# fdb/frequensea

Measured on AMD Instinct MI355X. Metric: fft_frames_per_sec_n8192, higher is better.
Workload: dtype f32

## Files before the change

### frequensea_amd/csrc/fsea_configs.h

```cpp
#pragma once

#include "fsea_opt.h"

#define FSEA_CFG_32 32, 4, 64, 2, 2, 8, 4, 1, 1, true, true, 0, fo::STREAMING_PIXELS | fo::WIN_DC_REGS
#define FSEA_CFG_64 64, 4, 64, 2, 2, 16, 4, 1, 1, true, true, 0, fo::STREAMING_PIXELS | fo::WIN_DC_REGS
#define FSEA_CFG_128 128, 4, 64, 2, 2, 16, 8, 1, 1, true, true, 0, fo::STREAMING_PIXELS | fo::WIN_DC_REGS
#define FSEA_CFG_256 256, 8, 32, 2, 2, 16, 16, 1, 1, true, true, 0, fo::STREAMING_PIXELS | fo::WIN_DC_REGS
#define FSEA_CFG_512 512, 16, 16, 2, 2, 32, 16, 1, 1, true, true, 0, fo::STREAMING_PIXELS | fo::WIN_DC_REGS
#define FSEA_CFG_1024 1024, 32, 8, 2, 3, 8, 16, 8, 1, true, true, 0, fo::STREAMING_PIXELS | fo::BALANCE_MAG | fo::WIN_DC_REGS_MAG | fo::LD_NT | fo::DEFER | fo::LANE_ROT | fo::TW_FUSE | fo::TW_HOIST | fo::BATCH_READS
#define FSEA_CFG_2048 2048, 64, 4, 2, 3, 16, 16, 8, 1, true, true, 0, fo::STREAMING_PIXELS | fo::BALANCE_MAG | fo::WIN_DC_REGS_MAG | fo::LD_NT | fo::LANE_ROT | fo::TW_FUSE | fo::TW_HOIST | fo::BATCH_READS
#define FSEA_CFG_4096 4096, 128, 2, 2, 3, 16, 16, 16, 1, true, true, 0, fo::STREAMING_PIXELS | fo::BALANCE_MAG | fo::LD_NT | fo::DEFER | fo::LANE_ROT_LAST | fo::LANE_ROT | fo::TW_FUSE | fo::TW_HOIST | fo::BATCH_READS
#define FSEA_CFG_8192 8192, 256, 1, 2, 3, 16, 16, 32, 1, true, true, 0, fo::STREAMING_PIXELS | fo::BALANCE_MAG | fo::WIN_DC_REGS | fo::LD_NT | fo::DEFER | fo::LANE_ROT | fo::TW_FUSE | fo::TW_HOIST | fo::BATCH_READS
#define FSEA_CFG_16384 16384, 512, 1, 2, 3, 16, 32, 32, 1, true, true, 0, fo::STREAMING_PIXELS | fo::WIN_DC_REGS_MAG | fo::LD_NT | fo::DEFER | fo::TW_FUSE

#define FSEA_CFG_256_ROWS 256, 8, 32, 2, 3, 4, 8, 8, 1, true, true, 0, fo::STREAMING_PIXELS | fo::WIN_DC_REGS | fo::LD_NT | fo::DEFER | fo::LANE_ROT | fo::TW_FUSE | fo::TW_HOIST | fo::BATCH_READS
#define FSEA_CFG_512_PX 512, 16, 16, 2, 2, 16, 32, 1, 1, true, true, 0, fo::STREAMING_PIXELS | fo::WIN_DC_REGS | fo::LD_NT | fo::TW_FUSE | fo::BATCH_READS
#define FSEA_CFG_1024_RT 1024, 32, 8, 2, 2, 32, 32, 1, 1, true, true, 0, fo::STREAMING_PIXELS | fo::WIN_DC_REGS | fo::TW_FUSE | fo::BATCH_READS

#define FSEA_WIN 2
```

### frequensea_amd/csrc/fsea_configs_tune.h

```cpp
#pragma once

#include "fsea_configs.h"

#define FSEA_CFG_8192_ND 8192, 256, 1, 2, 3, 16, 16, 32, 1, true, true, 0, fo::LANE_ROT | fo::TW_FUSE | fo::TW_HOIST | fo::BATCH_READS
#define FSEA_CFG_16384_ND 16384, 512, 1, 2, 3, 16, 32, 32, 1, true, true, 0, fo::TW_FUSE
#define FSEA_CFG_4096_DF 4096, 256, 1, 4, 3, 16, 16, 16, 1, true, true, 0, fo::DEFER | fo::TW_FUSE | fo::BATCH_READS
#define FSEA_CFG_2048_DF 2048, 64, 4, 2, 3, 16, 16, 8, 1, true, true, 0, fo::DEFER | fo::TW_FUSE | fo::TW_HOIST | fo::BATCH_READS
#define FSEA_CFG_8192_CP0 8192, 256, 1, 2, 3, 16, 16, 32, 1, true, true, 0, fo::DEFER | fo::LANE_ROT | fo::TW_FUSE | fo::TW_HOIST | fo::BATCH_READS
#define FSEA_CFG_8192_STNT 8192, 256, 1, 2, 3, 16, 16, 32, 1, true, true, 0, fo::ST_NT | fo::DEFER | fo::LANE_ROT | fo::TW_FUSE | fo::TW_HOIST | fo::BATCH_READS
#define FSEA_CFG_8192_LDNT 8192, 256, 1, 2, 3, 16, 16, 32, 1, true, true, 0, fo::LD_NT | fo::DEFER | fo::LANE_ROT | fo::TW_FUSE | fo::TW_HOIST | fo::BATCH_READS
#define FSEA_CFG_16384_CP0 16384, 512, 1, 2, 3, 16, 32, 32, 1, true, true, 0, fo::DEFER | fo::TW_FUSE
#define FSEA_CFG_16384_STNT 16384, 512, 1, 2, 3, 16, 32, 32, 1, true, true, 0, fo::ST_NT | fo::DEFER | fo::TW_FUSE
#define FSEA_CFG_4096_CP0 4096, 128, 2, 2, 3, 16, 16, 16, 1, true, true, 0, fo::DEFER | fo::LANE_ROT | fo::TW_FUSE | fo::TW_HOIST | fo::BATCH_READS
#define FSEA_CFG_4096_STNT 4096, 128, 2, 2, 3, 16, 16, 16, 1, true, true, 0, fo::ST_NT | fo::DEFER | fo::LANE_ROT | fo::TW_FUSE | fo::TW_HOIST | fo::BATCH_READS
#define FSEA_CFG_2048_CP0 2048, 64, 4, 2, 3, 16, 16, 8, 1, true, true, 0, fo::TW_FUSE | fo::TW_HOIST | fo::BATCH_READS
#define FSEA_CFG_2048_STNT 2048, 64, 4, 2, 3, 16, 16, 8, 1, true, true, 0, fo::ST_NT | fo::TW_FUSE | fo::TW_HOIST | fo::BATCH_READS
#define FSEA_CFG_1024_CP0 1024, 32, 8, 2, 2, 32, 32, 1, 1, true, true, 0, fo::TW_FUSE | fo::BATCH_READS
#define FSEA_CFG_1024_LDSTNT 1024, 32, 8, 2, 2, 32, 32, 1, 1, true, true, 0, fo::LD_NT | fo::ST_NT | fo::TW_FUSE | fo::BATCH_READS
#define FSEA_CFG_256_CP0 256, 8, 32, 2, 2, 16, 16, 1, 1, true, true, 0, 0
#define FSEA_CFG_256_LDSTNT 256, 8, 32, 2, 2, 16, 16, 1, 1, true, true, 0, fo::LD_NT | fo::ST_NT
#define FSEA_CFG_8192_V2 8192, 256, 1, 2, 3, 16, 16, 32, 1, true, true, 0, fo::V2 | fo::TW_FUSE | fo::BATCH_READS
#define FSEA_CFG_8192_V2S 8192, 256, 1, 2, 3, 16, 16, 32, 1, true, true, fsea::abl::V2_STATIC, fo::V2 | fo::TW_FUSE | fo::BATCH_READS
#define FSEA_CFG_8192_V2L 8192, 256, 1, 2, 3, 16, 16, 32, 1, true, true, fsea::abl::V2_V1_LOADS, fo::V2 | fo::TW_FUSE | fo::BATCH_READS
#define FSEA_CFG_8192_V2SL 8192, 256, 1, 2, 3, 16, 16, 32, 1, true, true, fsea::abl::V2_V1_LOADS | fsea::abl::V2_STATIC, fo::V2 | fo::TW_FUSE | fo::BATCH_READS
#define FSEA_CFG_8192_V2NA 8192, 256, 1, 2, 3, 16, 16, 32, 1, true, true, fsea::abl::V2_NO_EXCHANGE_A, fo::V2 | fo::TW_FUSE | fo::BATCH_READS
#define FSEA_CFG_8192_B2 8192, 256, 1, 2, 3, 16, 32, 16, 1, true, true, 0, fo::LD_NT | fo::ST_NT | fo::DEFER | fo::LANE_ROT | fo::TW_FUSE | fo::TW_HOIST | fo::BATCH_READS
#define FSEA_CFG_8192_D2 8192, 256, 1, 2, 3, 8, 32, 32, 1, true, true, 0, fo::LD_NT | fo::ST_NT | fo::DEFER | fo::LANE_ROT | fo::TW_FUSE | fo::TW_HOIST | fo::BATCH_READS
#define FSEA_CFG_8192_W 8192, 256, 1, 2, 3, 32, 32, 8, 1, true, true, 0, fo::LD_NT | fo::ST_NT | fo::DEFER | fo::LANE_ROT | fo::TW_FUSE | fo::TW_HOIST | fo::BATCH_READS
#define FSEA_CFG_8192_W2 8192, 256, 1, 2, 3, 32, 32, 8, 1, true, true, 0, fo::ST_NT | fo::DEFER | fo::LANE_ROT | fo::TW_FUSE | fo::TW_HOIST | fo::BATCH_READS
#define FSEA_CFG_8192_A 8192, 256, 1, 2, 3, 32, 16, 16, 1, true, true
#define FSEA_CFG_8192_B 8192, 256, 1, 2, 3, 16, 32, 16, 1, true, true
#define FSEA_CFG_8192_D 8192, 256, 1, 2, 3, 8, 32, 32, 1, true, true
#define FSEA_CFG_8192_NOTWL 8192, 256, 1, 2, 3, 16, 32, 16, 1, false, true
#define FSEA_CFG_8192_NOTWR 8192, 256, 1, 2, 3, 16, 32, 16, 1, true, false
#define FSEA_CFG_1024_B 1024, 64, 4, 4, 3, 16, 16, 4, 1, true, true
#define FSEA_CFG_1024_C 1024, 64, 4, 4, 3, 4, 16, 16, 1, true, true
#define FSEA_CFG_1024_D 1024, 32, 4, 2, 2, 32, 32, 1, 1, true, true
#define FSEA_CFG_4096_B 4096, 128, 2, 2, 3, 16, 16, 16, 1, true, true
#define FSEA_CFG_4096_C 4096, 128, 2, 2, 3, 16, 8, 32, 1, true, true
#define FSEA_CFG_4096_D 4096, 128, 2, 2, 3, 8, 16, 32, 1, true, true
#define FSEA_CFG_256_P16 256, 16, 16, 2, 2, 16, 16, 1, 1, true, true, 0, fo::ST_NT
#define FSEA_CFG_128_P16 128, 8, 32, 2, 2, 16, 8, 1, 1, true, true, 0, fo::ST_NT
#define FSEA_CFG_4096_T256 4096, 256, 1, 4, 3, 16, 16, 16, 1, true, true, 0, fo::LD_NT | fo::ST_NT | fo::TW_FUSE | fo::BATCH_READS
#define FSEA_CFG_4096_F1 4096, 128, 1, 2, 3, 16, 16, 16, 1, true, true, 0, fo::LD_NT | fo::ST_NT | fo::DEFER | fo::LANE_ROT | fo::TW_FUSE | fo::TW_HOIST | fo::BATCH_READS
#define FSEA_CFG_4096_B3 4096, 128, 2, 2, 3, 16, 16, 16, 1, true, true, 0, fo::LD_NT | fo::ST_NT | fo::LANE_ROT | fo::TW_FUSE | fo::TW_HOIST | fo::BATCH_READS
#define FSEA_CFG_4096_LR 4096, 128, 2, 2, 3, 16, 16, 16, 1, true, true, 0, fo::LD_NT | fo::ST_NT | fo::DEFER | fo::LANE_ROT | fo::TW_FUSE | fo::TW_HOIST | fo::BATCH_READS
#define FSEA_CFG_2048_LR 2048, 64, 4, 2, 3, 16, 16, 8, 1, true, true, 0, fo::LD_NT | fo::ST_NT | fo::TW_FUSE | fo::TW_HOIST | fo::BATCH_READS
#define FSEA_CFG_16384_B 16384, 512, 1, 2, 3, 32, 32, 16, 1, true, true
#define FSEA_CFG_2048_B 2048, 64, 4, 2, 3, 8, 8, 32, 1, true, true
#define FSEA_CFG_2048_C 2048, 64, 4, 2, 3, 4, 16, 32, 1, true, true
#define FSEA_CFG_8192_NOST 8192, 256, 1, 2, 3, 16, 16, 32, 1, true, true, fsea::abl::NO_STORES, fo::LANE_ROT | fo::TW_FUSE | fo::TW_HOIST | fo::BATCH_READS
#define FSEA_CFG_8192_NOLDS 8192, 256, 1, 2, 3, 16, 16, 32, 1, true, true, fsea::abl::NO_LDS, fo::LANE_ROT | fo::TW_FUSE | fo::TW_HOIST | fo::BATCH_READS
#define FSEA_CFG_8192_NOFLOP 8192, 256, 1, 2, 3, 16, 16, 32, 1, true, true, fsea::abl::NO_FLOPS, fo::LANE_ROT | fo::TW_FUSE | fo::TW_HOIST | fo::BATCH_READS
#define FSEA_CFG_8192_IO 8192, 256, 1, 2, 3, 16, 16, 32, 1, true, true, fsea::abl::NO_FLOPS | fsea::abl::NO_LDS, fo::LANE_ROT | fo::TW_FUSE | fo::TW_HOIST | fo::BATCH_READS
#define FSEA_CFG_8192_VALU 8192, 256, 1, 2, 3, 16, 16, 32, 1, true, true, fsea::abl::NO_LDS | fsea::abl::NO_STORES, fo::LANE_ROT | fo::TW_FUSE | fo::TW_HOIST | fo::BATCH_READS
#define FSEA_CFG_8192_IONT 8192, 256, 1, 2, 3, 16, 16, 32, 1, true, true, fsea::abl::NO_FLOPS | fsea::abl::NO_LDS, fo::LD_NT | fo::ST_NT | fo::LANE_ROT | fo::TW_FUSE | fo::TW_HOIST | fo::BATCH_READS
#define FSEA_CFG_8192_NOLDSNT 8192, 256, 1, 2, 3, 16, 16, 32, 1, true, true, fsea::abl::NO_LDS, fo::LD_NT | fo::ST_NT | fo::LANE_ROT | fo::TW_FUSE | fo::TW_HOIST | fo::BATCH_READS
#define FSEA_CFG_8192_NOFLOPNT 8192, 256, 1, 2, 3, 16, 16, 32, 1, true, true, fsea::abl::NO_FLOPS, fo::LD_NT | fo::ST_NT | fo::LANE_ROT | fo::TW_FUSE | fo::TW_HOIST | fo::BATCH_READS
#define FSEA_CFG_8192_NOLOAD 8192, 256, 1, 2, 3, 16, 16, 32, 1, true, true, fsea::abl::NO_LOADS, fo::LANE_ROT | fo::TW_FUSE | fo::TW_HOIST | fo::BATCH_READS
#define FSEA_CFG_128_ST0 128, 4, 64, 2, 2, 16, 8, 1, 1, true, true, 0, 0
#define FSEA_CFG_256_ST0 256, 8, 32, 2, 2, 16, 16, 1, 1, true, true, 0, 0
#define FSEA_CFG_512_ST0 512, 16, 16, 2, 2, 32, 16, 1, 1, true, true, 0, 0
#define FSEA_CFG_1024_ST0 1024, 32, 8, 2, 2, 32, 32, 1, 1, true, true, 0, fo::TW_FUSE | fo::BATCH_READS
#define FSEA_CFG_4096_PXNOLOG 4096, 128, 2, 2, 3, 16, 16, 16, 1, true, true, fsea::abl::NO_EPILOGUE_MATH, fo::LD_NT | fo::ST_NT | fo::DEFER | fo::LANE_ROT | fo::TW_FUSE | fo::TW_HOIST | fo::BATCH_READS
#define FSEA_CFG_4096_PXNOST 4096, 128, 2, 2, 3, 16, 16, 16, 1, true, true, fsea::abl::NO_STORES, fo::LD_NT | fo::ST_NT | fo::DEFER | fo::LANE_ROT | fo::TW_FUSE | fo::TW_HOIST | fo::BATCH_READS
#define FSEA_CFG_4096_PXIO 4096, 128, 2, 2, 3, 16, 16, 16, 1, true, true, fsea::abl::NO_FLOPS | fsea::abl::NO_LDS, fo::LD_NT | fo::ST_NT | fo::LANE_ROT | fo::TW_FUSE | fo::TW_HOIST | fo::BATCH_READS
#define FSEA_CFG_8192_PXNOLOG 8192, 256, 1, 2, 3, 16, 16, 32, 1, true, true, fsea::abl::NO_EPILOGUE_MATH, fo::LD_NT | fo::ST_NT | fo::DEFER | fo::LANE_ROT | fo::TW_FUSE | fo::TW_HOIST | fo::BATCH_READS
#define FSEA_CFG_8192_NOMAG 8192, 256, 1, 2, 3, 16, 16, 32, 1, true, true, fsea::abl::NO_EPILOGUE_MATH, fo::LANE_ROT | fo::TW_FUSE | fo::TW_HOIST | fo::BATCH_READS
#define FSEA_CFG_8192_X0 8192, 256, 1, 2, 3, 16, 16, 32, 1, true, true, 0, 0
#define FSEA_CFG_4096_X0 4096, 128, 2, 2, 3, 16, 16, 16, 1, true, true, 0, 0
#define FSEA_CFG_2048_X0 2048, 64, 4, 2, 3, 16, 16, 8, 1, true, true, 0, 0
#define FSEA_CFG_1024_X0 1024, 32, 8, 2, 2, 32, 32, 1, 1, true, true, 0, 0
#define FSEA_CFG_4096_W64 4096, 64, 1, 1, 2, 64, 64, 1, 1, false, false, 0, fo::W64 | fo::LD_NT | fo::ST_NT | fo::BATCH_READS
#define FSEA_CFG_4096_S2 4096, 64, 1, 1, 3, 16, 16, 16, 1, true, true, 0, fo::LD_NT | fo::ST_NT | fo::DEFER | fo::LANE_ROT | fo::TW_FUSE | fo::TW_HOIST | fo::BATCH_READS
#define FSEA_CFG_4096_W64B 4096, 64, 1, 1, 2, 64, 64, 1, 1, false, false, 0, fo::PX_BIAS | fo::W64 | fo::LD_NT | fo::ST_NT | fo::BATCH_READS
#define FSEA_CFG_4096_PK 4096, 128, 2, 2, 3, 16, 16, 16, 1, true, true, 0, fo::PX_PACK | fo::LD_NT | fo::ST_NT | fo::DEFER | fo::LANE_ROT_LAST | fo::LANE_ROT | fo::TW_FUSE | fo::TW_HOIST | fo::BATCH_READS
#define FSEA_CFG_4096_PX0 4096, 128, 2, 2, 3, 16, 16, 16, 1, true, true, 0, fo::LD_NT | fo::ST_NT | fo::DEFER | fo::LANE_ROT_LAST | fo::LANE_ROT | fo::TW_FUSE | fo::TW_HOIST | fo::BATCH_READS
#define FSEA_CFG_8192_PK 8192, 256, 1, 2, 3, 16, 16, 32, 1, true, true, 0, fo::PX_PACK | fo::LD_NT | fo::ST_NT | fo::DEFER | fo::LANE_ROT | fo::TW_FUSE | fo::TW_HOIST | fo::BATCH_READS
#define FSEA_CFG_8192_PX0 8192, 256, 1, 2, 3, 16, 16, 32, 1, true, true, 0, fo::LD_NT | fo::ST_NT | fo::DEFER | fo::LANE_ROT | fo::TW_FUSE | fo::TW_HOIST | fo::BATCH_READS
#define FSEA_CFG_256_PK 256, 8, 32, 2, 2, 16, 16, 1, 1, true, true, 0, fo::PX_PACK | fo::ST_NT
#define FSEA_CFG_256_PX0 256, 8, 32, 2, 2, 16, 16, 1, 1, true, true, 0, fo::ST_NT
#define FSEA_CFG_1024_PX0 1024, 32, 8, 2, 2, 32, 32, 1, 1, true, true, 0, fo::ST_NT | fo::TW_FUSE | fo::BATCH_READS
#define FSEA_CFG_1024_R2 FSEA_CFG_1024_RT
#define FSEA_CFG_256_P64 256, 4, 16, 1, 2, 16, 16, 1, 1, true, true, 0, fo::ST_NT
#define FSEA_CFG_4096_T256PX 4096, 256, 1, 4, 3, 16, 16, 16, 1, true, true, 0, fo::STREAMING_PIXELS | fo::LD_NT | fo::TW_FUSE | fo::BATCH_READS
#define FSEA_CFG_4096_F1PX 4096, 128, 1, 2, 3, 16, 16, 16, 1, true, true, 0, fo::STREAMING_PIXELS | fo::LD_NT | fo::DEFER | fo::LANE_ROT | fo::TW_FUSE | fo::TW_HOIST | fo::BATCH_READS
#define FSEA_CFG_32_C2 32, 4, 64, 2, 2, 4, 8, 1, 1, true, true, 0, fo::STREAMING_PIXELS
#define FSEA_CFG_64_C2 64, 4, 64, 2, 2, 8, 8, 1, 1, true, true, 0, fo::STREAMING_PIXELS
#define FSEA_CFG_64_T2 64, 2, 128, 2, 2, 8, 8, 1, 1, true, true, 0, fo::STREAMING_PIXELS
#define FSEA_CFG_1024_E 1024, 32, 8, 2, 3, 16, 8, 8, 1, true, true, 0, fo::STREAMING_PIXELS | fo::LD_NT | fo::LANE_ROT | fo::TW_FUSE | fo::TW_HOIST | fo::BATCH_READS
#define FSEA_CFG_1024_F 1024, 32, 8, 2, 3, 8, 16, 8, 1, true, true, 0, fo::STREAMING_PIXELS | fo::LD_NT | fo::LANE_ROT | fo::TW_FUSE | fo::TW_HOIST | fo::BATCH_READS
#define FSEA_CFG_1024_G 1024, 32, 8, 2, 3, 16, 16, 4, 1, true, true, 0, fo::STREAMING_PIXELS | fo::LD_NT | fo::LANE_ROT | fo::TW_FUSE | fo::TW_HOIST | fo::BATCH_READS
#define FSEA_CFG_1024_H 1024, 32, 8, 2, 3, 8, 8, 16, 1, true, true, 0, fo::STREAMING_PIXELS | fo::LD_NT | fo::LANE_ROT | fo::TW_FUSE | fo::TW_HOIST | fo::BATCH_READS
#define FSEA_CFG_1024_FD 1024, 32, 8, 2, 3, 8, 16, 8, 1, true, true, 0, fo::STREAMING_PIXELS | fo::LD_NT | fo::DEFER | fo::LANE_ROT | fo::TW_FUSE | fo::TW_HOIST | fo::BATCH_READS
#define FSEA_CFG_1024_F0 1024, 32, 8, 2, 3, 8, 16, 8, 1, true, true, 0, fo::STREAMING_PIXELS | fo::LD_NT | fo::TW_FUSE | fo::TW_HOIST | fo::BATCH_READS
#define FSEA_CFG_1024_FL 1024, 32, 8, 2, 3, 8, 16, 8, 1, true, true, 0, fo::STREAMING_PIXELS | fo::LANE_ROT | fo::TW_FUSE | fo::TW_HOIST | fo::BATCH_READS
#define FSEA_CFG_512_888 512, 16, 16, 2, 3, 8, 8, 8, 1, true, true, 0, fo::STREAMING_PIXELS | fo::LD_NT | fo::DEFER | fo::LANE_ROT | fo::TW_FUSE | fo::TW_HOIST | fo::BATCH_READS
#define FSEA_CFG_512_1632 FSEA_CFG_512_PX
#define FSEA_CFG_256_488 FSEA_CFG_256_ROWS
#define FSEA_CFG_256_884 256, 8, 32, 2, 3, 8, 8, 4, 1, true, true, 0, fo::STREAMING_PIXELS | fo::LD_NT | fo::DEFER | fo::LANE_ROT | fo::TW_FUSE | fo::TW_HOIST | fo::BATCH_READS
#define FSEA_CFG_128_448 128, 4, 64, 2, 3, 4, 4, 8, 1, true, true, 0, fo::STREAMING_PIXELS | fo::LD_NT | fo::DEFER | fo::LANE_ROT | fo::TW_FUSE | fo::TW_HOIST | fo::BATCH_READS
#define FSEA_CFG_2048_81616 2048, 64, 4, 2, 3, 8, 16, 16, 1, true, true, 0, fo::STREAMING_PIXELS | fo::LD_NT | fo::DEFER | fo::LANE_ROT | fo::TW_FUSE | fo::TW_HOIST | fo::BATCH_READS
#define FSEA_CFG_4096_16328 4096, 128, 2, 2, 3, 16, 32, 8, 1, true, true, 0, fo::STREAMING_PIXELS | fo::LD_NT | fo::DEFER | fo::LANE_ROT_LAST | fo::LANE_ROT | fo::TW_FUSE | fo::TW_HOIST | fo::BATCH_READS
// ... 13 lines not shown
```

### frequensea_amd/csrc/fsea_fft_core.h

```cpp
#pragma once

#include <hip/hip_runtime.h>
#include <stddef.h>
#include <stdint.h>

#include <fsea_pk_asm.h>
#include "fsea_opt.h"
#ifdef FSEA_TUNE
#include <fsea_pk_asm_tune.h>
#endif

namespace fsea {

constexpr int ilog2c(int n) {
    int l = 0;
    while ((1 << l) < n) ++l;
    return l;
}

constexpr int bitrev_c(int i, int bits) {
    int r = 0;
    for (int b = 0; b < bits; ++b) {
        if (i & (1 << b)) r |= 1 << (bits - 1 - b);
    }
// ... 120 lines not shown
        y[bitrev_c(i, BITS)] = plus;
        y[bitrev_c(i + R / 2, BITS)] = cf_fma(a, cf{2.0f, 2.0f}, -plus);
    }
    dft_const_levels<R, 2>(y);
#pragma unroll
    for (int i = 0; i < R; ++i) x[i * S] = y[i];
}

template <int R, int HALF, int TS, int DROP = 0>
__device__ __forceinline__ void dft_def_level(cf *y, const cf *tw) {
    if constexpr (HALF < R) {
        constexpr int OFF = HALF / 2, DISTINCT = HALF >= 2 ? HALF / 2 : 1;
#pragma unroll
        for (int base = 0; base < R; base += 2 * HALF) {
#pragma unroll
            for (int k = 0; k < DISTINCT; ++k) {
                cf &a = y[base + k], &b = y[base + k + HALF];
                const cf plus = pk_cmul_add(b, tw[(OFF + k) * TS], a);
                if constexpr (HALF <= DROP) b = a;
                else b = cf_fma(a, cf{2.0f, 2.0f}, -plus);
                a = plus;
            }
            if constexpr (HALF >= 2) {
#pragma unroll
                for (int k = 0; k < DISTINCT; ++k) {
                    cf &a = y[base + DISTINCT + k], &b = y[base + DISTINCT + k + HALF];
                    const cf plus = pk_cmul_add_mi(b, tw[(OFF + k) * TS], a);
                    if constexpr (HALF <= DROP) b = a;
                    else b = cf_fma(a, cf{2.0f, 2.0f}, -plus);
                    a = plus;
                }
            }
        }
        dft_def_level<R, 2 * HALF, TS, DROP>(y, tw);
    }
}

template <int R, int S, int TS, int DROP = 0>
__device__ __forceinline__ void dft_regs_def(cf *x, const cf *tw) {
    static_assert(R >= 4 && R <= 64 && (R & (R - 1)) == 0, "radix must be 4..64");
    constexpr int BITS = ilog2c(R);
    cf y[R];
#pragma unroll
    for (int i = 0; i < R; ++i) y[bitrev_c(i, BITS)] = x[i * S];
    dft_def_level<R, 1, TS, DROP>(y, tw);
#pragma unroll
    for (int i = 0; i < R; ++i) x[i * S] = y[i];
}

enum : int {
    MODE_MAG = 0,
    MODE_DB10_U8 = 1,
    MODE_DB5_U8_DCFIX = 2,
    MODE_COMPLEX = 3,
    MODE_MAG_NODC = 4,
    MODE_DB_F32 = 5
};
enum : int { IN_U8 = 0, IN_F32 = 1, IN_U8_ROT = 2 };

#ifndef FSEA_DEFAULT_OPT
#define FSEA_DEFAULT_OPT 0
#endif
#ifndef FSEA_STATIC_CONTIG
#define FSEA_STATIC_CONTIG 0
#endif
#ifndef FSEA_TRACE
#define FSEA_TRACE 0
#endif

template <int N_, int T_, int FPW_, int WPE_, int NP_, int R0_, int R1_, int R2_ = 1, int R3_ = 1,
          bool TWL_ = true, bool TWR_ = true, int ABL_ = 0, int OPT_ = FSEA_DEFAULT_OPT>
struct FftCfg {
    static constexpr int OPT = OPT_;
    static constexpr int ABL = ABL_;
    static constexpr int N = N_, T = T_, FPW = FPW_, NP = NP_;
    static constexpr int WPE = WPE_;
    static constexpr int P = N_ / T_;
    static constexpr int WG = T_ * FPW_;
    static constexpr bool TWL = TWL_, TWR = TWR_;
    static constexpr int R(int i) { return i == 0 ? R0_ : i == 1 ? R1_ : i == 2 ? R2_ : R3_; }
    static constexpr int C(int i) { return P / R(i); }
    static constexpr int Ns(int i) { return i == 0 ? 1 : Ns(i - 1) * R(i - 1); }
    static constexpr int tw_len(int i) { return i == 0 ? 0 : (R(i) - 1) * Ns(i); }
    static constexpr int pad(int idx) { return lds_pad<N_ / T_>(idx); }
    static constexpr int LDS_FRAME = N_ + 2 * T_;
    static constexpr int lds_tw_off(int i) {
        return i <= 1 ? FPW_ * LDS_FRAME : lds_tw_off(i - 1) + tw_len(i - 1);
    }
    static constexpr int TAB_MID = lds_tw_off(NP_ - 1) - FPW_ * LDS_FRAME;
    static constexpr int TAB_HI = N_ >= 64 ? N_ / 64 : 1, TAB_LO = 64;
    static constexpr int TAB_SMALL = TAB_MID + (TWR_ ? TAB_HI + TAB_LO : 0);
    static constexpr int LDS_HI = FPW_ * LDS_FRAME + TAB_MID;
    static constexpr int LDS_LO = LDS_HI + TAB_HI;
    static constexpr int LDS_TOTAL = FPW_ * LDS_FRAME + ((TWL_ || TWR_) ? TAB_SMALL : 0);
    static constexpr int LDS_ALLOC = LDS_TOTAL + 2;
    static_assert(R0_ * R1_ * R2_ * R3_ == N_, "radices must multiply to N");
    static_assert(N_ % T_ == 0, "T must divide N");
    static_assert(NP_ >= 2 && NP_ <= 4, "2..4 passes");
};

struct FftArgs {
    const void *in;
    void *out;
    size_t n_frames;
    size_t hop;
    uint32_t xormask;
    int mode;
    unsigned *ctr;
    unsigned long long *trace;
    const cf *tw[4];
    const cf *tw_small;
    const cf *tw_def;
    double rot_delta, rot_phase0;
    cf rot_row[32];
    uint32_t tile_rows = 0, pitch_row = 0, pitch_tile = 0;
    size_t out_span = 0;
    uint32_t dynamic_units = 1;
    uint32_t run_len = 0;
    const float *win = nullptr;
    const cf *win_dc = nullptr;
    uint32_t win_offset = 0;
};

template <int C>
__device__ __forceinline__ void ld_c(const cf *p, cf *dst) {
    if constexpr (C == 1) {
        dst[0] = *p;
    } else {
#pragma unroll
        for (int c = 0; c < C; c += 2) {
            const cf2 q = *reinterpret_cast<const cf2 *>(p + c);
            dst[c] = cf{q[0], q[1]};
            dst[c + 1] = cf{q[2], q[3]};
        }
    }
}

template <int C>
__device__ __forceinline__ void st_c(cf *p, const cf *src) {
    if constexpr (C == 1) {
        *p = src[0];
    } else {
#pragma unroll
        for (int c = 0; c < C; c += 2) {
            *reinterpret_cast<cf2 *>(p + c) = cf2{src[c][0], src[c][1], src[c + 1][0], src[c + 1][1]};
        }
    }
}

typedef __amdgpu_buffer_rsrc_t rsrc_t;

__device__ __forceinline__ rsrc_t buffer_window(const void *base, size_t off, size_t total) {
    const size_t rem = total > off ? total - off : 0;
    char *p = const_cast<char *>(static_cast<const char *>(base)) + (rem ? off : 0);
    return __builtin_amdgcn_make_buffer_rsrc(p, 0, rem > 0xffffffffull ? 0xffffffffu : (uint32_t)rem, 0x00020000);
}

typedef uint32_t u32x2 __attribute__((vector_size(8)));
typedef uint32_t u32x4 __attribute__((vector_size(16)));

__device__ __forceinline__ uint32_t f2u(float x) { return __builtin_bit_cast(uint32_t, x); }
__device__ __forceinline__ float u2f(uint32_t x) { return __builtin_bit_cast(float, x); }

#ifndef FSEA_STORE_GUARD
#define FSEA_STORE_GUARD 1
#endif
__device__ __forceinline__ void store_data_guard() {
#if !defined(__AMDGCN__)
// ... 109 lines not shown
            const uint32_t w = words[q] ^ xormask;
            dst[2 * q] = cf{b2f(w, 0), b2f(w, 1)};
            const cf odd = cf{b2f(w, 2), b2f(w, 3)};
            dst[2 * q + 1] = SIGNED ? -odd : odd;
        }
    }
}

__device__ __forceinline__ cf turn_phasor_f64(double turns) {
    turns -= floor(turns);
    double s, c;
    sincospi(2.0 * turns, &s, &c);
    return cf{(float)c, (float)s};
}
__device__ __forceinline__ cf turn_phasor_f32(double turns) {
    turns -= floor(turns);
    float s, c;
    sincospif(2.0f * (float)turns, &s, &c);
    return cf{c, s};
}

template <class Cfg, int IN, int MODE_T = -1, bool ROT = false, bool RUNS = false, int WIN = 0>
struct FftKernel {
    static_assert(!ROT || IN == IN_U8, "the fused frequency shift is a u8-input path");
    static_assert(WIN == 0 || (Cfg::TWR && (Cfg::OPT & opt::TUNE_ONLY) == 0 && Cfg::P >= 8),
                  "the windowed kernels: V1 schedule, register-resident last-pass twiddles");
    static_assert(WIN == 0 || !RUNS || (IN == IN_U8 && !ROT), "windowed half-overlap runs: the plain u8 kernel only");
    static constexpr bool WIN_DC = WIN != 0 && IN == IN_U8;
    static constexpr bool LATE_LOAD = WIN != 0 && IN == IN_F32;
    static constexpr bool DC_IN_REGS = WIN_DC && ((Cfg::OPT & opt::WIN_DC_REGS) != 0 ||
                                                  ((Cfg::OPT & opt::WIN_DC_REGS_MAG) != 0 && MODE_T == MODE_MAG && !ROT));
    static_assert(!RUNS || (IN == IN_U8 && !ROT && Cfg::FPW == 1 && (Cfg::R(0) % 2) == 0), "half-overlap runs: u8 input, one frame per workgroup");
    static constexpr int N = Cfg::N, T = Cfg::T, P = Cfg::P, NP = Cfg::NP, FPW = Cfg::FPW;
    static constexpr int LAST = NP - 1;
    static constexpr int R0 = Cfg::R(0), C0 = Cfg::C(0);
    static constexpr int RL = Cfg::R(LAST), CL = Cfg::C(LAST), NsL = Cfg::Ns(LAST);
    static constexpr bool ONE_WAVE = (Cfg::WG <= 64) || (T <= 64 && (64 % T) == 0);
    static constexpr float SC = (IN == IN_U8) ? (1.0f / 256.0f) : 1.0f;
    static constexpr bool PRESCALED = Cfg::TWR && (IN == IN_U8);
    using Raw = RawRow<IN, C0>;
    static constexpr bool BATCH_READS = (Cfg::OPT & opt::BATCH_READS) != 0;
    static constexpr bool TW_HOIST = (Cfg::OPT & opt::TW_HOIST) != 0;
    static constexpr bool TW_FUSE = (Cfg::OPT & opt::TW_FUSE) != 0 && (Cfg::ABL & abl::NO_FLOPS) == 0;
    static constexpr int ST_AUX = (Cfg::OPT & opt::ST_NT) ? 2 : 0;
    template <int ELEM_BYTES>
    static constexpr int st_aux() { return (T * CL * ELEM_BYTES >= 128 && CL * ELEM_BYTES <= 16) ? ST_AUX : (ST_AUX & ~2); }
    static constexpr int LD_AUX = (Cfg::OPT & opt::LD_NT) ? 2 : 0;
    static constexpr bool DEFER = (Cfg::OPT & opt::DEFER) != 0 && NP == 3;
    static constexpr bool PX_PACK = (Cfg::OPT & opt::PX_PACK) != 0;
    static constexpr bool PX_BIAS = (Cfg::OPT & opt::PX_BIAS) != 0;
    static constexpr bool LANE_ROT = (Cfg::OPT & opt::LANE_ROT) != 0;
    static constexpr bool LANE_ROT_LAST = (Cfg::OPT & opt::LANE_ROT_LAST) != 0;
    template <int I>
    static __device__ __forceinline__ int pass_lane(int t) {
        constexpr bool ON = (I == LAST) ? LANE_ROT_LAST : LANE_ROT;
        if constexpr (ON && Cfg::C(I) == 2 && P == 32 && (T % 16) == 0) {
            const int blk = t >> 4;
            return (blk << 4) | ((t - blk) & 15);
        } else if constexpr (ON && Cfg::C(I) == 1 && P == 16 && T == 256) {
            const int blk = t >> 4;
            const int logical = (blk >> 1) | ((blk & 1) << 3);
            return (logical << 4) | (t & 15);
        } else {
            return t;
        }
    }

    static __device__ __forceinline__ void after_reads() {
        if constexpr (BATCH_READS) __builtin_amdgcn_sched_barrier(0);
    }

    static __device__ __forceinline__ void frame_sync() {
        if constexpr (Cfg::ABL & abl::NO_LDS) {
            return;
        } else if constexpr (ONE_WAVE) {
            __builtin_amdgcn_fence(__ATOMIC_RELEASE, "wavefront");
            __builtin_amdgcn_wave_barrier();
            __builtin_amdgcn_fence(__ATOMIC_ACQUIRE, "wavefront");
        } else {
            __syncthreads();
        }
    }

    static constexpr uint32_t IN_BPS = (IN == IN_U8) ? 2 : 8;

    static __device__ __forceinline__ void load_raw(rsrc_t rs, uint32_t voff, Raw *raw) { load_raw_rows<0, R0>(rs, voff, raw); }

    template <int RLO, int RHI>
    static __device__ __forceinline__ void load_raw_rows(rsrc_t rs, uint32_t voff, Raw *raw) {
        constexpr int STRIDE = N / R0;
#pragma unroll
        for (int r = RLO; r < RHI; ++r) {
            const uint32_t soff = (uint32_t)(r * STRIDE) * IN_BPS;
            if constexpr (IN == IN_U8) {
                if constexpr (C0 == 1) raw[r].w = __builtin_amdgcn_raw_buffer_load_b16(rs, voff, soff, LD_AUX);
                if constexpr (C0 == 2) raw[r].w = __builtin_amdgcn_raw_buffer_load_b32(rs, voff, soff, LD_AUX);
                if constexpr (C0 == 4) {
                    const auto q = __builtin_amdgcn_raw_buffer_load_b64(rs, voff, soff, LD_AUX);
                    raw[r].w.x = q[0];
                    raw[r].w.y = q[1];
                }
                if constexpr (C0 == 8) {
                    const auto q = __builtin_amdgcn_raw_buffer_load_b128(rs, voff, soff, LD_AUX);
                    raw[r].w.x = q[0];
                    raw[r].w.y = q[1];
                    raw[r].w.z = q[2];
                    raw[r].w.w = q[3];
                }
            } else if constexpr (C0 == 1) {
                const auto q = __builtin_amdgcn_raw_buffer_load_b64(rs, voff, soff, LD_AUX);
                raw[r].w[0] = cf{u2f(q[0]), u2f(q[1])};
            } else {
#pragma unroll
                for (int c = 0; c < C0; c += 2) {
                    const auto q = __builtin_amdgcn_raw_buffer_load_b128(rs, voff + 8 * c, soff, LD_AUX);
                    raw[r].w[c] = cf{u2f(q[0]), u2f(q[1])};
                    raw[r].w[c + 1] = cf{u2f(q[2]), u2f(q[3])};
                }
            }
        }
    }

    template <int I>
    static __device__ __forceinline__ void apply_twiddles(cf *v, const cf *tw, int t) {
        constexpr int R = Cfg::R(I), C = Cfg::C(I), Ns = Cfg::Ns(I);
        const int k0 = (C * t) % Ns;
#pragma unroll
        for (int r = 1; r < R; ++r) {
            cf w[C];
            if constexpr (Ns % C == 0) {
                ld_c<C>(tw + (r - 1) * Ns + k0, w);
            } else {
#pragma unroll
                for (int c = 0; c < C; ++c) w[c] = tw[(r - 1) * Ns + (C * t + c) % Ns];
            }
#pragma unroll
            for (int c = 0; c < C; ++c) {
                if constexpr (Cfg::ABL & abl::NO_FLOPS) v[r * C + c] += w[c];
                else v[r * C + c] = pk_cmul(v[r * C + c], w[c]);
            }
        }
    }

    template <int I>
    static __device__ __forceinline__ void lds_write(cf *lds, const cf *v, int t) {
        constexpr int R = Cfg::R(I), C = Cfg::C(I), Ns = Cfg::Ns(I);
        if constexpr (Cfg::ABL & abl::NO_LDS) {
            return;
        } else if constexpr (Ns == 1 && (R % 2) == 0) {
            cf *base = lds + (unsigned)((P + 2) * t);
#pragma unroll
            for (int c = 0; c < C; ++c) {
#pragma unroll
                for (int r = 0; r < R; r += 2) {
                    const cf pr[2] = {v[r * C + c], v[(r + 1) * C + c]};
                    st_c<2>(base + (c * R + r), pr);
                }
            }
        } else if constexpr (Ns % C == 0) {
            const unsigned j = (unsigned)(C * t);
            const unsigned j0 = (j / Ns) * (Ns * R) + (j % Ns);
            if constexpr (Ns % P == 0) {
                cf *base = lds + Cfg::pad(j0);
#pragma unroll
                for (int r = 0; r < R; ++r) st_c<C>(base + r * (Ns + 2 * (Ns / P)), v + r * C);
            } else {
                constexpr int Q = P / Ns;
                static_assert(P % Ns == 0 && R % Q == 0, "pad addressing needs Ns | P and (P/Ns) | R");
#pragma unroll
                for (int b = 0; b < Q; ++b) {
                    cf *base = lds + Cfg::pad(j0 + b * Ns);
#pragma unroll
                    for (int rq = 0; rq < R / Q; ++rq) st_c<C>(base + rq * (P + 2), v + (rq * Q + b) * C);
                }
            }
        } else {
#pragma unroll
            for (int c = 0; c < C; ++c) {
                const int j = C * t + c;
                const int j0 = (j / Ns) * (Ns * R) + (j % Ns);
#pragma unroll
                for (int r = 0; r < R; ++r) lds[Cfg::pad(j0 + r * Ns)] = v[r * C + c];
            }
        }
    }

    template <int I>
    static __device__ __forceinline__ void lds_read(const cf *lds, cf *v, int t) {
        constexpr int R = Cfg::R(I), C = Cfg::C(I);
        constexpr int STRIDE = N / R;
        if constexpr (Cfg::ABL & abl::NO_LDS) {
            return;
        } else if constexpr (STRIDE % P == 0) {
            const cf *base = lds + Cfg::pad(C * t);
#pragma unroll
            for (int r = 0; r < R; ++r) ld_c<C>(base + r * (STRIDE + 2 * (STRIDE / P)), v + r * C);
        } else {
#pragma unroll
            for (int r = 0; r < R; ++r) ld_c<C>(lds + Cfg::pad(C * t + r * STRIDE), v + r * C);
        }
    }

    template <int I>
    static __device__ __forceinline__ void middle_pass(cf *lds, const cf *lds_all, cf *v, const FftArgs &a, int t0,
                                                       const cf *tw_res = nullptr) {
        if constexpr (I < LAST) {
            constexpr int R = Cfg::R(I), C = Cfg::C(I);
            const int t = pass_lane<I>(t0);
            const cf *tw = Cfg::TWL ? (lds_all + Cfg::lds_tw_off(I)) : a.tw[I];
            if constexpr (DEFER) {
                lds_read<I>(lds, v, t);
                after_reads();
                frame_sync();
#pragma unroll
                for (int c = 0; c < C; ++c) dft_regs_def<R, C, 1, (Cfg::ABL & abl::DROP_32_OPS) ? 2 : ((Cfg::ABL & abl::DROP_16_OPS) ? 1 : 0)>(v + c, tw_res + c * (R / 2));
            } else if constexpr (TW_HOIST && (Cfg::Ns(I) % C == 0)) {
                constexpr int Ns = Cfg::Ns(I);
                cf w[(R - 1) * C];
                const int k0 = (C * t) % Ns;
#pragma unroll
                for (int r = 1; r < R; ++r) ld_c<C>(tw + (r - 1) * Ns + k0, w + (r - 1) * C);
                lds_read<I>(lds, v, t);
                after_reads();
                frame_sync();
                if constexpr (TW_FUSE) {
#pragma unroll
                    for (int c = 0; c < C; ++c) dft_regs_tw<R, C, C>(v + c, w + c, 1.0f);
                } else {
#pragma unroll
                    for (int r = 1; r < R; ++r) {
#pragma unroll
                        for (int c = 0; c < C; ++c) v[r * C + c] = pk_cmul(v[r * C + c], w[(r - 1) * C + c]);
                    }
                }
            } else {
                lds_read<I>(lds, v, t);
                after_reads();
                frame_sync();
                apply_twiddles<I>(v, tw, t);
            }
            if constexpr (!DEFER && !(TW_FUSE && TW_HOIST && (Cfg::Ns(I) % C == 0))) {
#pragma unroll
                for (int c = 0; c < C; ++c) dft_regs<R, C, (Cfg::ABL & abl::NO_FLOPS) != 0>(v + c);
            }
            lds_write<I>(lds, v, t);
            frame_sync();
            middle_pass<I + 1>(lds, lds_all, v, a, t0, tw_res);
        }
    }

    static __device__ __forceinline__ uint32_t elem_bytes(int mode) {
        return (mode == MODE_DB10_U8 || mode == MODE_DB5_U8_DCFIX) ? 1u : (mode == MODE_COMPLEX ? 8u : 4u);
    }

    static __device__ __forceinline__ float bin_power(const cf *v, int r, int c) {
        const cf z = v[r * CL + c];
        return __builtin_fmaf(z[0], z[0], z[1] * z[1]);
    }

    static __device__ __forceinline__ void epilogue(int mode, rsrc_t out, uint32_t lane_elem, cf *v, int t) {
        constexpr float SE = PRESCALED ? 1.0f : SC;
        constexpr float SE2 = SE * SE;
        const bool patched = (mode == MODE_MAG) || (mode == MODE_DB5_U8_DCFIX);
        if (WIN == 0 && IN == IN_U8 && !patched && t == 0) {
            const float dc = (PRESCALED ? 0.5f : 128.0f) * (float)N;
            v[(RL / 2) * CL] += cf{dc, dc};
        }
        if (mode == MODE_COMPLEX) {
            const uint32_t voff = lane_elem * 8u;
#pragma unroll
            for (int r = 0; r < RL; ++r) {
                cf z[CL];
#pragma unroll
                for (int c = 0; c < CL; ++c) z[c] = v[r * CL + c] * cf{SE, SE};
                bst<CL, st_aux<8>()>(out, voff, (uint32_t)(r * NsL) * 8u, z);
            }
        } else if (mode == MODE_DB10_U8 || mode == MODE_DB5_U8_DCFIX) {
            const float kdb = (mode == MODE_DB10_U8 ? 100.0f : 50.0f) * 0.30102999566398120f;
            const uint32_t voff = lane_elem;
#pragma unroll
            for (int r = 0; r < RL; ++r) {
                const uint32_t soff = (uint32_t)(r * NsL);
                uint8_t px[CL];
                [[maybe_unused]] uint32_t pxw[(CL + 3) / 4] = {};
#pragma unroll
                for (int c = 0; c < CL; ++c) {
                    float p = bin_power(v, r, c);
                    if constexpr (!PRESCALED && IN == IN_U8) p *= SE2;
                    if constexpr (PX_PACK) {
                        float d;
                        if constexpr (PX_BIAS) d = __builtin_fmaf(kdb, __builtin_amdgcn_logf(p), -0.49999997f);
                        else d = trunc_f32(kdb * __builtin_amdgcn_logf(p));
                        if constexpr (Cfg::ABL & abl::NO_EPILOGUE_MATH) d = kdb * p;
                        pxw[c / 4] = cvt_pk_u8(d, (uint32_t)(c & 3), pxw[c / 4]);
                    } else {
                        float d = kdb * __builtin_amdgcn_logf(p);
                        if constexpr (Cfg::ABL & abl::NO_EPILOGUE_MATH) d = kdb * p;
                        int q = (int)d;
                        q = q < 0 ? 0 : (q > 255 ? 255 : q);
                        px[c] = (uint8_t)q;
                    }
                }
                if constexpr (PX_PACK) {
#pragma unroll
                    for (int c = 0; c < CL; ++c) px[c] = (uint8_t)(pxw[c / 4] >> (8 * (c & 3)));
                }
                if constexpr (Cfg::ABL & abl::NO_STORES) {
                    if (px[0] == 255 && px[CL - 1] == 254 && v[0][0] == -1.0f) bst<CL>(out, voff, soff, px);
                } else if (patched && r == RL / 2 && t == 0) {
#pragma unroll
                    for (int c = 1; c < CL; ++c) bst<1>(out, voff + c, soff, px + c);
                } else if constexpr (PX_PACK) {
                    if constexpr (CL == 1) __builtin_amdgcn_raw_buffer_store_b8((uint8_t)pxw[0], out, voff, soff, st_aux<1>());
                    else if constexpr (CL == 2) __builtin_amdgcn_raw_buffer_store_b16((uint16_t)pxw[0], out, voff, soff, st_aux<1>());
                    else {
#pragma unroll
                        for (int c = 0; c < CL; c += 4) __builtin_amdgcn_raw_buffer_store_b32(pxw[c / 4], out, voff + c, soff, st_aux<1>());
                    }
                } else {
                    bst<CL, st_aux<1>()>(out, voff, soff, px);
                }
// ... 454 lines not shown
```

### frequensea_amd/csrc/fsea_opt.h

```cpp
#pragma once

namespace fsea {
namespace opt {
enum : int {
    BATCH_READS = 2,
    TW_HOIST = 4,
    TW_FUSE = 8,
    LANE_ROT = 16,
    LANE_ROT_LAST = 32,
    DEFER = 128,
    ST_NT = 4096,
    LD_NT = 32768,
    PX_PACK = 2097152,
    PX_BIAS = 4194304,
    WIN_DC_REGS = 16777216,
    BALANCE_PX = 67108864,
    BALANCE_MAG = 134217728,
    WIN_DC_REGS_MAG = 33554432,
    V2 = 64,
    W64 = 1048576,
    PW = 8388608,
    TUNE_ONLY = V2 | W64 | PW,
    STREAMING_PIXELS = ST_NT | PX_PACK | PX_BIAS | BALANCE_PX,
};
}
namespace abl {
enum : int {
    NO_STORES = 1,
    NO_LDS = 2,
    NO_FLOPS = 4,
    V2_STATIC = 8, V2_V1_LOADS = 16, V2_NO_EXCHANGE_A = 32,
    NO_LOADS = 64,
    NO_EPILOGUE_MATH = 128,
    DROP_16_OPS = 256,
    DROP_32_OPS = 512,
};
}
}
namespace fo = fsea::opt;
```

### frequensea_amd/csrc/k_tune_8192b.hip

```cpp
#include "fsea_configs_tune.h"
#include "fsea_registry.h"
FSEA_DEFINE_KERNEL_LITE(fsea_fft8192x0, "x0", FSEA_CFG_8192_X0)
FSEA_DEFINE_KERNEL_LITE(fsea_fft8192v2, "v2", FSEA_CFG_8192_V2)
FSEA_DEFINE_KERNEL_LITE(fsea_fft8192v2s, "v2s", FSEA_CFG_8192_V2S)
FSEA_DEFINE_KERNEL_LITE(fsea_fft8192stnt, "st_nt", FSEA_CFG_8192_STNT)
FSEA_DEFINE_KERNEL_LITE(fsea_fft8192ldnt, "ld_nt", FSEA_CFG_8192_LDNT)
FSEA_DEFINE_KERNEL_LITE(fsea_fft8192cp0, "cp0", FSEA_CFG_8192_CP0)
FSEA_REGISTER_BEGIN(tune_8192b)
FSEA_REGISTER(fsea_fft8192x0)
FSEA_REGISTER(fsea_fft8192v2)
FSEA_REGISTER(fsea_fft8192v2s)
FSEA_REGISTER(fsea_fft8192stnt)
FSEA_REGISTER(fsea_fft8192ldnt)
FSEA_REGISTER(fsea_fft8192cp0)
FSEA_REGISTER_END
```

Measured before the change: 81.90 million.

## Make last LDS exchange in-place to drop a barrier in 8192 FFT

Adds an X2_INPLACE option that gives the second-to-last pass an LDS layout with per-row shifts, so each lane's last-pass reads touch only slots it wrote itself. The frame_sync between reads and writes in the penultimate pass can then be skipped. The option is enabled for the default 8192 config, and the old layout is kept as a tune variant. It adds extra LDS per frame and more complex address math, and it relies on static-assert preconditions for correctness.

```diff
diff --git a/frequensea_amd/csrc/fsea_configs.h b/frequensea_amd/csrc/fsea_configs.h
--- a/frequensea_amd/csrc/fsea_configs.h
+++ b/frequensea_amd/csrc/fsea_configs.h
@@ -10,7 +10,7 @@
 #define FSEA_CFG_1024 1024, 32, 8, 2, 3, 8, 16, 8, 1, true, true, 0, fo::STREAMING_PIXELS | fo::BALANCE_MAG | fo::WIN_DC_REGS_MAG | fo::LD_NT | fo::DEFER | fo::LANE_ROT | fo::TW_FUSE | fo::TW_HOIST | fo::BATCH_READS
 #define FSEA_CFG_2048 2048, 64, 4, 2, 3, 16, 16, 8, 1, true, true, 0, fo::STREAMING_PIXELS | fo::BALANCE_MAG | fo::WIN_DC_REGS_MAG | fo::LD_NT | fo::LANE_ROT | fo::TW_FUSE | fo::TW_HOIST | fo::BATCH_READS
 #define FSEA_CFG_4096 4096, 128, 2, 2, 3, 16, 16, 16, 1, true, true, 0, fo::STREAMING_PIXELS | fo::BALANCE_MAG | fo::LD_NT | fo::DEFER | fo::LANE_ROT_LAST | fo::LANE_ROT | fo::TW_FUSE | fo::TW_HOIST | fo::BATCH_READS
-#define FSEA_CFG_8192 8192, 256, 1, 2, 3, 16, 16, 32, 1, true, true, 0, fo::STREAMING_PIXELS | fo::BALANCE_MAG | fo::WIN_DC_REGS | fo::LD_NT | fo::DEFER | fo::LANE_ROT | fo::TW_FUSE | fo::TW_HOIST | fo::BATCH_READS
+#define FSEA_CFG_8192 8192, 256, 1, 2, 3, 16, 16, 32, 1, true, true, 0, fo::X2_INPLACE | fo::STREAMING_PIXELS | fo::BALANCE_MAG | fo::WIN_DC_REGS | fo::LD_NT | fo::DEFER | fo::LANE_ROT | fo::TW_FUSE | fo::TW_HOIST | fo::BATCH_READS
 #define FSEA_CFG_16384 16384, 512, 1, 2, 3, 16, 32, 32, 1, true, true, 0, fo::STREAMING_PIXELS | fo::WIN_DC_REGS_MAG | fo::LD_NT | fo::DEFER | fo::TW_FUSE
 
 #define FSEA_CFG_256_ROWS 256, 8, 32, 2, 3, 4, 8, 8, 1, true, true, 0, fo::STREAMING_PIXELS | fo::WIN_DC_REGS | fo::LD_NT | fo::DEFER | fo::LANE_ROT | fo::TW_FUSE | fo::TW_HOIST | fo::BATCH_READS
diff --git a/frequensea_amd/csrc/fsea_configs_tune.h b/frequensea_amd/csrc/fsea_configs_tune.h
--- a/frequensea_amd/csrc/fsea_configs_tune.h
+++ b/frequensea_amd/csrc/fsea_configs_tune.h
@@ -19,6 +19,7 @@
 #define FSEA_CFG_1024_LDSTNT 1024, 32, 8, 2, 2, 32, 32, 1, 1, true, true, 0, fo::LD_NT | fo::ST_NT | fo::TW_FUSE | fo::BATCH_READS
 #define FSEA_CFG_256_CP0 256, 8, 32, 2, 2, 16, 16, 1, 1, true, true, 0, 0
 #define FSEA_CFG_256_LDSTNT 256, 8, 32, 2, 2, 16, 16, 1, 1, true, true, 0, fo::LD_NT | fo::ST_NT
+#define FSEA_CFG_8192_X2OFF 8192, 256, 1, 2, 3, 16, 16, 32, 1, true, true, 0, fo::STREAMING_PIXELS | fo::BALANCE_MAG | fo::WIN_DC_REGS | fo::LD_NT | fo::DEFER | fo::LANE_ROT | fo::TW_FUSE | fo::TW_HOIST | fo::BATCH_READS
 #define FSEA_CFG_8192_V2 8192, 256, 1, 2, 3, 16, 16, 32, 1, true, true, 0, fo::V2 | fo::TW_FUSE | fo::BATCH_READS
 #define FSEA_CFG_8192_V2S 8192, 256, 1, 2, 3, 16, 16, 32, 1, true, true, fsea::abl::V2_STATIC, fo::V2 | fo::TW_FUSE | fo::BATCH_READS
 #define FSEA_CFG_8192_V2L 8192, 256, 1, 2, 3, 16, 16, 32, 1, true, true, fsea::abl::V2_V1_LOADS, fo::V2 | fo::TW_FUSE | fo::BATCH_READS
diff --git a/frequensea_amd/csrc/fsea_fft_core.h b/frequensea_amd/csrc/fsea_fft_core.h
--- a/frequensea_amd/csrc/fsea_fft_core.h
+++ b/frequensea_amd/csrc/fsea_fft_core.h
@@ -226,8 +226,23 @@
     static constexpr int C(int i) { return P / R(i); }
     static constexpr int Ns(int i) { return i == 0 ? 1 : Ns(i - 1) * R(i - 1); }
     static constexpr int tw_len(int i) { return i == 0 ? 0 : (R(i) - 1) * Ns(i); }
-    static constexpr int pad(int idx) { return lds_pad<N_ / T_>(idx); }
-    static constexpr int LDS_FRAME = N_ + 2 * T_;
+    static constexpr bool X2 = (OPT_ & opt::X2_INPLACE) != 0;
+    static constexpr int X2_ROWLEN = X2 ? N_ / R(NP_ - 2) : N_;
+    static constexpr int X2_SHIFT = X2 ? Ns(NP_ - 2) : 0;
+    static constexpr int X2_PITCH = X2_ROWLEN + 2 * (X2_ROWLEN / (N_ / T_));
+    __host__ __device__ static constexpr int x2_row_shift(int row) { return X2 ? row * X2_SHIFT : 0; }
+    __host__ __device__ static constexpr int x2_mid_slot(int t, int r) {
+        return lds_pad<N_ / T_>(C(NP_ - 2) * t) + r * X2_PITCH + x2_row_shift(r);
+    }
+    __host__ __device__ static constexpr int x2_last_base(int k) {
+        return (k / Ns(NP_ - 2)) * X2_PITCH + x2_row_shift(k / Ns(NP_ - 2)) + k % Ns(NP_ - 2);
+    }
+    __host__ __device__ static constexpr int x2_last_off(int a) { return lds_pad<N_ / T_>(a * Ns(NP_ - 2)); }
+    __host__ __device__ static constexpr int pad(int idx) {
+        if constexpr (X2) return lds_pad<N_ / T_>(idx) + x2_row_shift(idx / X2_ROWLEN);
+        else return lds_pad<N_ / T_>(idx);
+    }
+    static constexpr int LDS_FRAME = N_ + 2 * T_ + (X2 ? (R(NP_ - 2) - 1) * X2_SHIFT : 0);
     static constexpr int lds_tw_off(int i) {
         return i <= 1 ? FPW_ * LDS_FRAME : lds_tw_off(i - 1) + tw_len(i - 1);
     }
@@ -503,6 +518,14 @@
         }
     }
 
+    template <int I>
+    static __device__ __forceinline__ void reads_done() {
+        if constexpr (!(Cfg::X2 && I == LAST - 1)) frame_sync();
+    }
+    static_assert(!Cfg::X2 || (NP == 3 && CL == 1 && Cfg::X2_ROWLEN % P == 0 && P % Cfg::Ns(1) == 0 && Cfg::Ns(1) == 16 &&
+                               (Cfg::X2_PITCH % 32) == 0 && (Cfg::OPT & opt::TUNE_ONLY) == 0),
+                  "in-place second exchange: three passes, one bin per lane in the last, rows of whole 256-byte bank rows");
+
     static constexpr uint32_t IN_BPS = (IN == IN_U8) ? 2 : 8;
 
     static __device__ __forceinline__ void load_raw(rsrc_t rs, uint32_t voff, Raw *raw) { load_raw_rows<0, R0>(rs, voff, raw); }
@@ -568,8 +591,12 @@
         constexpr int R = Cfg::R(I), C = Cfg::C(I), Ns = Cfg::Ns(I);
         if constexpr (Cfg::ABL & abl::NO_LDS) {
             return;
+        } else if constexpr (Cfg::X2 && I == LAST - 1) {
+#pragma unroll
+            for (int r = 0; r < R; ++r) st_c<C>(lds + Cfg::x2_mid_slot(t, r), v + r * C);
         } else if constexpr (Ns == 1 && (R % 2) == 0) {
             cf *base = lds + (unsigned)((P + 2) * t);
+            if constexpr (Cfg::X2) base += Cfg::x2_row_shift((P * t) / Cfg::X2_ROWLEN);
 #pragma unroll
             for (int c = 0; c < C; ++c) {
 #pragma unroll
@@ -612,6 +639,16 @@
         constexpr int STRIDE = N / R;
         if constexpr (Cfg::ABL & abl::NO_LDS) {
             return;
+        } else if constexpr (Cfg::X2 && I == LAST - 1) {
+#pragma unroll
+            for (int r = 0; r < R; ++r) ld_c<C>(lds + Cfg::x2_mid_slot(t, r), v + r * C);
+        } else if constexpr (Cfg::X2 && I == LAST) {
+            const cf *base = lds + Cfg::x2_last_base(t);
+#pragma unroll
+            for (int r = 0; r < R; ++r) {
+                ld_c<1>(base + Cfg::x2_last_off(r), v + r);
+                asm volatile("" ::: "memory");
+            }
         } else if constexpr (STRIDE % P == 0) {
             const cf *base = lds + Cfg::pad(C * t);
 #pragma unroll
@@ -632,7 +669,7 @@
             if constexpr (DEFER) {
                 lds_read<I>(lds, v, t);
                 after_reads();
-                frame_sync();
+                reads_done<I>();
 #pragma unroll
                 for (int c = 0; c < C; ++c) dft_regs_def<R, C, 1, (Cfg::ABL & abl::DROP_32_OPS) ? 2 : ((Cfg::ABL & abl::DROP_16_OPS) ? 1 : 0)>(v + c, tw_res + c * (R / 2));
             } else if constexpr (TW_HOIST && (Cfg::Ns(I) % C == 0)) {
@@ -643,7 +680,7 @@
                 for (int r = 1; r < R; ++r) ld_c<C>(tw + (r - 1) * Ns + k0, w + (r - 1) * C);
                 lds_read<I>(lds, v, t);
                 after_reads();
-                frame_sync();
+                reads_done<I>();
                 if constexpr (TW_FUSE) {
 #pragma unroll
                     for (int c = 0; c < C; ++c) dft_regs_tw<R, C, C>(v + c, w + c, 1.0f);
@@ -657,7 +694,7 @@
             } else {
                 lds_read<I>(lds, v, t);
                 after_reads();
-                frame_sync();
+                reads_done<I>();
                 apply_twiddles<I>(v, tw, t);
             }
             if constexpr (!DEFER && !(TW_FUSE && TW_HOIST && (Cfg::Ns(I) % C == 0))) {
diff --git a/frequensea_amd/csrc/fsea_opt.h b/frequensea_amd/csrc/fsea_opt.h
--- a/frequensea_amd/csrc/fsea_opt.h
+++ b/frequensea_amd/csrc/fsea_opt.h
@@ -17,6 +17,7 @@
     BALANCE_PX = 67108864,
     BALANCE_MAG = 134217728,
     WIN_DC_REGS_MAG = 33554432,
+    X2_INPLACE = 268435456,
     V2 = 64,
     W64 = 1048576,
     PW = 8388608,
diff --git a/frequensea_amd/csrc/k_tune_8192b.hip b/frequensea_amd/csrc/k_tune_8192b.hip
--- a/frequensea_amd/csrc/k_tune_8192b.hip
+++ b/frequensea_amd/csrc/k_tune_8192b.hip
@@ -6,6 +6,7 @@
 FSEA_DEFINE_KERNEL_LITE(fsea_fft8192stnt, "st_nt", FSEA_CFG_8192_STNT)
 FSEA_DEFINE_KERNEL_LITE(fsea_fft8192ldnt, "ld_nt", FSEA_CFG_8192_LDNT)
 FSEA_DEFINE_KERNEL_LITE(fsea_fft8192cp0, "cp0", FSEA_CFG_8192_CP0)
+FSEA_DEFINE_KERNEL_LITE(fsea_fft8192x2off, "x2off", FSEA_CFG_8192_X2OFF)
 FSEA_REGISTER_BEGIN(tune_8192b)
 FSEA_REGISTER(fsea_fft8192x0)
 FSEA_REGISTER(fsea_fft8192v2)
@@ -13,4 +14,5 @@
 FSEA_REGISTER(fsea_fft8192stnt)
 FSEA_REGISTER(fsea_fft8192ldnt)
 FSEA_REGISTER(fsea_fft8192cp0)
+FSEA_REGISTER(fsea_fft8192x2off)
 FSEA_REGISTER_END
```

After: 82.68 million, median of 6. About the same (+1.0%).
